# shmurthy08/MoE-GAN_CPSC541

Measured on AMD Instinct MI355X. Metric: images/sec (G+D step, 64x64 MS-COCO layout), higher is better.
Workload: dtype bf16; 1 GPU; C2: 64x64, 8 experts top-2, batch 256/GPU, bf16, R1 on; global_batch=256, experts=8, topk=2, parallelism=dp1, world_seen=1, launch=hipGraph replay

## Files before the change

### include/moegan_hip.h

```cpp
#ifndef MOEGAN_HIP_H
#define MOEGAN_HIP_H
#include <stddef.h>
#include <stdint.h>

#ifdef __cplusplus
extern "C" {
#endif

#define MG_OK 0
#define MG_ERR_ARG (-1)
#define MG_ERR_LAUNCH (-2)

#define MG_F32 0
#define MG_BF16 1
#define MG_F32X3 2

#define MG_ACT_NONE 0
#define MG_ACT_LRELU 1
#define MG_ACT_GELU 2
#define MG_ACT_MUL_GELU_GRAD 3
#define MG_ACT_MUL_LRELU_GRAD 4
#define MG_ACT_RSQRT_EPS 5
#define MG_ACT_QUICK_GELU 6
#define MG_ACT_MUL_QUICK_GELU_GRAD 7
// ... 3 lines not shown
  const float* bias;
  const float* scale;
  int32_t scale_shift;
  int64_t scale_ld;
  const float* rowscale;
  int32_t act;
  const void* aux;
  int64_t ld_aux;
  const void* resid;
  int64_t ld_res;
  int32_t accumulate;
  int32_t atomic;
  int32_t remap_lgcin;
  int32_t remap_taps;
  const int32_t* a_idx;
  int32_t a_idx_div;
  const float* a_rowscale;
  int32_t a_gelu;
  const float* addvec;
  int32_t add_shift;
  int64_t add_ld;
  void* out_pre;
  int64_t ld_pre;
} mg_epilogue;

const char* mg_last_error(void);
int mg_version(void);
const char* mg_source_hash(void);

int mg_set_workspace(void* ptr, size_t bytes, void* stream);
int mg_workspace_reserve(size_t bytes, void* stream);
int64_t mg_workspace_bytes(void* stream);
int mg_set_tuning(int key, int value);

int mg_timer_event_create(void** event);
int mg_timer_event_record(void* event, void* stream);
int mg_timer_event_elapsed(void* start, void* stop, float* ms);
int mg_timer_event_destroy(void* event);
int mg_mark(int tag, void* stream);

typedef struct mg_gemm_desc {
  int32_t M, N, K;
  const void* A;
  int64_t lda;
  const void* B;
  int64_t ldb;
// ... 91 lines not shown
int mg_disc_head_sum(const float* P, int B, int Hf, float* out, void* stream);

int mg_disc_head_bwd_data(int dtype, const float* g, int64_t g_bstride, const float* W2, const void* a1, int B, int Hf, int Cf, int out_dtype, void* ga1, void* stream);

int mg_disc_head_bwd_w(int dtype, const float* g, int64_t g_bstride, const void* h1, int B, int Hf, int Cf, float* dW2, void* stream);

int mg_d_loss(const float* img_real, const float* img_fake, const float* tb, const int32_t* perm, int B, int No, int Nf, float* out, float* g_img, float* g_fake, float* g_tb, float* real_out, float* mism_out, float* fake_out, void* stream);

int mg_g_loss(const float* fake, int B, float scale, float* out, float* g, void* stream);

int mg_r1(int dtype, const void* g, int64_t per, int B, float gamma, float* r1, int u_dtype, void* u, void* stream);

int mg_lrelu_mask_mul(int a_dtype, const void* a, int m_dtype, const void* m, int64_t n, int out_dtype, void* out, void* stream);

int mg_segsum(int dtype, const void* X, int64_t ld, int B, int HW, int C, float* out, void* stream);

int mg_modconv_bwd_out(int dtype, int gz_dtype, const void* gz, int64_t ld_gz, const void* z, int64_t ld_z, const void* zsub, int64_t ld_zsub, const float* d, int B, int HW, int Cout, int act, void* gyt, int64_t ld_gyt, float* gdd, void* stream);

int mg_gather_rows(int dtype, const void* src, int64_t lds, const int32_t* idx, int idx_div, const float* rowscale, int n, int C, void* out, int64_t ldo, void* stream);

int mg_scale_bc(int dtype, const void* x, int64_t ldx, const float* s, int64_t lds, int B, int HW, int C, void* out, int64_t ldo, void* stream);

int mg_modconv_bwd_in(int gxt_dtype, const void* gxt, int64_t ld_gxt, int dtype, const void* x, int64_t ld_x, const float* s, int64_t ld_s, int B, int HW, int Cin, int gx_dtype, void* gx, int64_t ld_gx, int accumulate, float* gs, void* stream);

int mg_kl_coefs(const float* kl2, int R, float eff_w, float* coef, float* total, void* stream);

int mg_router_reparam(const float* mu, const float* rho, const float* eps, int64_t n, float* W, void* stream);

int mg_router_fwd(int dtype, const void* tok, int64_t ld, int T, int C, const float* Wfc, const float* Lt, int E, int k, int HW, const float* temperature, float anneal, int eval_mode, float* probs, float* zlog, int32_t* topi, float* gate, void* stream);

int mg_moe_dispatch(const int32_t* topi, const float* gate, int T, int k, int E, int bm, int32_t* ws, int32_t* row_off, int32_t* tile_off, int32_t* perm, int32_t* pos_of, float* gate_pos, void* stream);

int mg_moe_combine(int dtype, const void* Y, int64_t ldy, const int32_t* pos_of, const float* gate, int T, int k, int C, const void* resid, int64_t ldr, void* out, int64_t ldo, void* stream);
int mg_moe_combine_scaled(int dtype, const void* Y, int64_t ldy, const int32_t* pos_of, const float* gate, int T, int k, int C, const void* resid, int64_t ldr, void* out, int64_t ldo, const float* s, int64_t lds, int HW, void* xs, int64_t ldxs, void* stream);

int mg_moe_gate_grad(int dtype, int gout_dtype, const void* gout, int64_t ldg, const void* Y, int64_t ldy, const int32_t* pos_of, int T, int k, int C, float* g_gate, void* stream);

int mg_router_bwd(const float* probs, const float* zlog, const int32_t* topi, const float* gate, const float* g_gate, const float* g_probs, const float* g_logits, const float* coef, int T, int E, int k, int HW, const float* temperature, float anneal, float* g_raw, float* gsum, float* g_temp, void* stream);

int mg_moe_token_grad(int dtype, const void* gX, int64_t ldx, const int32_t* pos_of, int T, int k, int C, const float* g_raw, const float* Wfc, int E, int out_dtype, void* out, int64_t ldo, void* stream);

int mg_router_feat_grad(int dtype, const void* tok, int64_t ld, int T, int C, const float* g_raw, int E, float* G1, void* stream);

int mg_grouped_colsum(int dtype, const void* X, int64_t ld, const int32_t* idx, int idx_div, const float* rs, const int32_t* row_off, int G, int N, int max_rows, float* out, void* stream);

int mg_router_kl(const float* mu_f, const float* rho_f, int nf, const float* mu_t, const float* rho_t, int nt, const float* mu_c, const float* rho_c, int nc, float* out, void* stream);
// ... 159 lines not shown
```

### moe-gan_cpsc541_amd/csrc/mg_common.h

```cpp
#pragma once
#include <hip/hip_runtime.h>
#include <stdint.h>

#include <algorithm>
#include <atomic>
#include <string>

#include "../../include/moegan_hip.h"

typedef uint16_t bf16_t;
typedef __bf16 bf16x8_t __attribute__((ext_vector_type(8)));
typedef unsigned short u16x8_t __attribute__((ext_vector_type(8)));
typedef unsigned short u16x4_t __attribute__((ext_vector_type(4)));
typedef float f32x4_t __attribute__((ext_vector_type(4)));

#define MG_DEV __device__ __forceinline__

MG_DEV float bf2f(bf16_t h) { return __uint_as_float(((uint32_t)h) << 16); }
MG_DEV bf16_t f2bf(float f) { return __builtin_bit_cast(bf16_t, (__bf16)f); }

MG_DEV float ldf(const float* p, int64_t i) { return p[i]; }
MG_DEV float ldf(const bf16_t* p, int64_t i) { return bf2f(p[i]); }
MG_DEV void stf(float* p, int64_t i, float v) { p[i] = v; }
MG_DEV void stf(bf16_t* p, int64_t i, float v) { p[i] = f2bf(v); }
// ... 105 lines not shown

void mg_set_error(const std::string& msg);
int mg_check_launch(const char* what);
enum { MG_TUNE_WGRAD_TILE = 0, MG_TUNE_GWGRAD_TILE = 1, MG_TUNE_CONV_TILE = 2, MG_TUNE_GEMM_TILE = 3,
       MG_TUNE_WGRAD_SPLITS = 4, MG_TUNE_NO_SLABS = 5, MG_TUNE_XCD = 6 , MG_TUNE_WGRAD_MODE = 7,
       MG_TUNE_WARP_LDS = 8, MG_TUNE_SHORTK = 9, MG_TUNE_ATOMIC_BLOCKS = 10, MG_TUNE_DETERMINISTIC = 11,
       MG_TUNE_S1_OFF = 12,
       MG_TUNE_D0_STORE = 13,
       MG_TUNE_FFN_BWD_OCC = 14,
       MG_TUNE_WIDE_WGRAD = 15,
       MG_TUNE_NARROW = 16,
       MG_TUNE_NARROW_BLOCKS = 17,
       MG_TUNE_DISPATCH3 = 18,
       MG_TUNE_NARROW_WPX = 19,
       MG_TUNE_GWGRAD_BLOCKS = 20,
       MG_TUNE_BATCH_SPLIT = 21,
       MG_TUNE_GROUPED_SHORTK = 22,
       MG_TUNE_SPLITK_FUSED = 23,
       MG_TUNE_ROUTER_TEAM = 24,
       MG_TUNE_ADAMW_CACHED = 25,
       MG_TUNE_ATOMIC_MINK = 26,
       MG_TUNE_WIDE_BLOCKS = 27,
       MG_TUNE_WGRAD_SLAB_BLOCKS = 28,
       MG_TUNE_COUNT = 29 };
extern std::atomic<int> g_mg_tune[MG_TUNE_COUNT];
inline bool mg_det() { return g_mg_tune[MG_TUNE_DETERMINISTIC].load(std::memory_order_relaxed) != 0; }
void* mg_workspace(size_t bytes, hipStream_t stream);
int* mg_tile_counters(int n, hipStream_t stream);
void* mg_fold_alloc(size_t bytes, hipStream_t stream);
int mg_fold_rows_submit(const mg_fold_rows& r, bool deferred, hipStream_t stream);
int mg_fold_wgrad_submit(const mg_fold_wgrad& r, bool deferred, hipStream_t stream);
inline float* mg_fold_partials(size_t bytes, hipStream_t st, bool* deferred) {
  void* p = mg_fold_alloc(bytes, st);
  *deferred = p != nullptr;
  return reinterpret_cast<float*>(p ? p : mg_workspace(bytes, st));
}

namespace {
__global__ __launch_bounds__(1024) void k_det_fold_rows(const float* __restrict__ part, int nrows, int ncols, int na,
                                                        float* __restrict__ out_a, float* __restrict__ out_b) {
  __shared__ float red[16][64];
  const int cx = threadIdx.x & 63, ry = threadIdx.x >> 6;
  const int i = blockIdx.x * 64 + cx;
  float s = 0.f;
  if (i < ncols)
    for (int r = ry; r < nrows; r += 16) s += part[(int64_t)r * ncols + i];
  red[ry][cx] = s;
// ... 19 lines not shown
}
static inline void mg_det_fold_rows(const float* part, int nrows, int ncols, int na, float* out_a, float* out_b,
                             hipStream_t st) {
  hipLaunchKernelGGL(k_det_fold_rows, dim3((ncols + 63) / 64), dim3(1024), 0, st, part, nrows, ncols, na, out_a, out_b);
}

#define MG_REQUIRE(cond, msg)                       \
  do {                                              \
    if (!(cond)) {                                  \
      mg_set_error(std::string(__func__) + ": " + (msg)); \
      return MG_ERR_ARG;                            \
    }                                               \
  } while (0)

static inline int cdiv(int64_t a, int64_t b) { return (int)((a + b - 1) / b); }

bool mg_conv3_direct_ok(int H, int W, int Cin, int Cout, int KH, int KW, int stride, int pad, bool wgrad);
bool mg_conv3_direct(const void* x, int B, int H, int Cin, const void* wpack, int Cout, const mg_epilogue* e, void* y,
                     int64_t ldy, int y_dtype, hipStream_t st);
bool mg_wgrad3_direct(const void* gy, int64_t ldg, const void* x, int B, int H, int Cin, float** ws_out, int* splits,
                      bool* deferred,
                      hipStream_t st);

bool mg_wgrad_wide(int M, int N, int K, const void* A, int64_t lda, const void* B, int64_t ldb, float* C, int64_t ldc,
                   float alpha, hipStream_t st);
```

### moe-gan_cpsc541_amd/csrc/mg_gemm.h

```cpp
#pragma once
#include <type_traits>

#include "mg_common.h"

namespace mg {


constexpr int NTHREADS = 256;
#ifndef MG_DB_MAX_TILE
#define MG_DB_MAX_TILE 0
#endif
#ifndef MG_NSTAGE
#define MG_NSTAGE 1
#endif
#ifndef MG_EPI_BLOCK_SYNC
#define MG_EPI_BLOCK_SYNC 0
#endif
#ifndef MG_SB2_MAX_TILE
#define MG_SB2_MAX_TILE 0
#endif
#ifndef MG_EPI_PREFETCH
#define MG_EPI_PREFETCH 1
#endif
#ifndef MG_SETPRIO
// ... 570 lines not shown
  }
  MG_DEV int pf_kind() const { return 1; }
  MG_DEV void pf_load(int m, int n, Pf& p) const {
    if (this->rm_mode == 1) m = this->remap_row(m);
    const TO* src = this->aux + (int64_t)m * this->ld_aux + n;
#pragma unroll
    for (int j = 0; j < Base::OV; ++j)
      p.v[j] = *reinterpret_cast<const typename Base::ovec_t*>(src + j * VecOf<TO>::N);
  }
  __attribute__((always_inline)) MG_DEV void vec8(int m, int n, float* v, const Pf* pf = nullptr) const {
    float t[8];
    if (pf) Base::pf_unpack(*pf, t);
    else ld8(this->aux + (int64_t)(this->rm_mode == 1 ? this->remap_row(m) : m) * this->ld_aux + n, t);
#pragma unroll
    for (int j = 0; j < 8; ++j) v[j] *= quick_gelu_grad(t[j]);
    Base::vec8(m, n, v, nullptr);
  }
  MG_DEV void operator()(int m, int n, float v) const {
    const int mm = this->rm_mode == 1 ? this->remap_row(m) : m;
    Base::operator()(m, n, v * quick_gelu_grad(ldf(this->aux, (int64_t)mm * this->ld_aux + n)));
  }
};

struct Grouping {
  int mode;
  int ngroups;
  const int* row_off;
  const int* tile_off;
  int rows_per_group;
  int swz;
  int sub_shift;
};

template <typename T> struct Tile;
template <> struct Tile<bf16_t> { static constexpr int BK = 64, PADK = 0, PADM = 32; };
template <> struct Tile<float> { static constexpr int BK = 32, PADK = 4, PADM = 16; };

#ifndef MG_BK_SMALL
#define MG_BK_SMALL 64
#endif
#ifndef MG_X3_BK
#define MG_X3_BK 64
#endif
template <typename T, bool X3, int BM = 128, int BN = 128> constexpr int tile_bk() {
  return X3 ? (BM * BN <= 64 * 64 ? MG_X3_BK : Tile<bf16_t>::BK)
            : (sizeof(T) == 2 && BM * BN <= 64 * 64) ? MG_BK_SMALL : Tile<T>::BK;
// ... 44 lines not shown
MG_DEV void epi_tile(const f32x4_t (&acc)[BM / 32][BN / 32], void* smem, const EP& ep, int m0, int n0, int Mloc,
                     int N, int mrow_base) {
  constexpr int WM = BM / 2, WN = BN / 2, FM = WM / 16, FN = WN / 16;
  const int tid = threadIdx.x, lane = tid & 63, wid = tid >> 6;
  const int wm = wid >> 1, wn = wid & 1;
  const int fr = lane & 15, fq = lane >> 4;
  constexpr int CSP = WN + 4;
  float* cs = reinterpret_cast<float*>(smem) + wid * 16 * CSP;
  constexpr int NE = (2 * WN + 63) / 64;
  constexpr bool kPf = PF && MG_EPI_PREFETCH && EP::OV == 1 && FM * NE * 4 <= 32;
  const bool pfp = kPf && ep.vec_ok && ep.pf_kind() != 0;
  typename EP::Pf pf[kPf ? FM : 1][kPf ? NE : 1];
  if constexpr (kPf) if (pfp) {
#pragma unroll
    for (int i = 0; i < FM; ++i)
#pragma unroll
      for (int t = 0; t < NE; ++t) {
        const int e = lane + 64 * t;
        const int rr = e / (WN / 8), cc = (e - rr * (WN / 8)) * 8;
        const int m = m0 + wm * WM + i * 16 + rr, n = n0 + wn * WN + cc;
        if (e < 2 * WN && m < Mloc && n + 8 <= N) ep.pf_load(mrow_base + m, n, pf[i][t]);
      }
  }
  __syncthreads();
#pragma unroll
  for (int i = 0; i < FM; ++i) {
    if (MG_EPI_BLOCK_SYNC) __syncthreads();
    else { __builtin_amdgcn_fence(__ATOMIC_SEQ_CST, "wavefront"); __builtin_amdgcn_wave_barrier(); }
#pragma unroll
    for (int j = 0; j < FN; ++j)
#pragma unroll
      for (int r = 0; r < 4; ++r) cs[(fq * 4 + r) * CSP + j * 16 + fr] = acc[i][j][r];
    if (MG_EPI_BLOCK_SYNC) __syncthreads();
    else { __builtin_amdgcn_fence(__ATOMIC_SEQ_CST, "wavefront"); __builtin_amdgcn_wave_barrier(); }
    const int mb = m0 + wm * WM + i * 16, nb = n0 + wn * WN;
    if (kPf && pfp) {
#pragma unroll
      for (int t = 0; t < (kPf ? NE : 0); ++t) {
        const int e = lane + 64 * t;
        const int rr = e / (WN / 8), cc = (e - rr * (WN / 8)) * 8;
        const int m = mb + rr, n = nb + cc;
        if (e >= 2 * WN || m >= Mloc) continue;
        const float* src = cs + rr * CSP + cc;
        if (n + 8 <= N) {
          float v[8];
          f32x4_t a = *reinterpret_cast<const f32x4_t*>(src), b = *reinterpret_cast<const f32x4_t*>(src + 4);
#pragma unroll
          for (int j = 0; j < 4; ++j) { v[j] = a[j]; v[j + 4] = b[j]; }
          ep.vec8(mrow_base + m, n, v, &pf[kPf ? i : 0][kPf ? t : 0]);
        } else {
          for (int j = 0; j < 8 && n + j < N; ++j) ep(mrow_base + m, n + j, src[j]);
        }
      }
    } else if (ep.vec_ok) {
#pragma unroll 1
      for (int e = lane; e < 2 * WN; e += 64) {
        int rr = e / (WN / 8), cc = (e - (e / (WN / 8)) * (WN / 8)) * 8;
        int m = mb + rr, n = nb + cc;
        if (m >= Mloc) continue;
        const float* src = cs + rr * CSP + cc;
        if (n + 8 <= N) {
          float v[8];
          f32x4_t a = *reinterpret_cast<const f32x4_t*>(src), b = *reinterpret_cast<const f32x4_t*>(src + 4);
#pragma unroll
          for (int j = 0; j < 4; ++j) { v[j] = a[j]; v[j + 4] = b[j]; }
          ep.vec8(mrow_base + m, n, v);
        } else {
          for (int j = 0; j < 8 && n + j < N; ++j) ep(mrow_base + m, n + j, src[j]);
        }
      }
    } else {
#pragma unroll 1
      for (int e = lane; e < 16 * WN; e += 64) {
        int rr = e / WN, cc = e - (e / WN) * WN;
        int m = mb + rr, n = nb + cc;
        if (m < Mloc && n < N) ep(mrow_base + m, n, cs[rr * CSP + cc]);
      }
    }
  }
}

template <typename T, int BM, int BN, bool A_KC, bool B_KC, class AL, class BL, class EP, bool X3 = false,
          bool PF = false>
MG_DEV void gemm_tile(const AL& A, const BL& B, const EP& ep, int m0, int n0, int Mloc, int N, int kbeg, int kend,
                      int mrow_base) {
  static_assert(!X3 || std::is_same<T, float>::value, "split-bf16 staging takes fp32 operands");
  constexpr int VEC = VecOf<T>::N;
  typedef typename VecOf<T>::type vec_t;
  typedef typename std::conditional<X3, bf16_t, T>::type LT;
  constexpr int TBK = tile_bk<T, X3, BM, BN>();
  constexpr int LDK = TBK + Tile<LT>::PADK;
  constexpr bool GMC = [] {
    if constexpr (!A_KC && !B_KC)
      return MG_GLDS_MC && !X3 && sizeof(T) == 2 && BM == BN && (BM == 64 || BM == 128) && TBK == 64 &&
             has_gldsmc<AL>::value && has_gldsmc<BL>::value;
    else return false;
  }();
  constexpr int PADMC = GMC ? 0 : Tile<LT>::PADM;
  constexpr int LDA = A_KC ? LDK : BM + PADMC;
  constexpr int LDB = B_KC ? LDK : BN + PADMC;
  constexpr int A_ELEMS = A_KC ? BM * LDK : TBK * LDA;
// ... 589 lines not shown
```

### moe-gan_cpsc541_amd/csrc/mg_gemm.hip

```cpp
#include <algorithm>
#include <string>
#include <type_traits>

#include "mg_gemm.h"
#include "mg_host.h"

using namespace mg;

namespace {


constexpr Grouping kNoGroup{0, 1, nullptr, nullptr, 0};
inline Grouping xcd_group() {
  Grouping g = kNoGroup;
  const int x = g_mg_tune[MG_TUNE_XCD];
  g.swz = x == 0 ? 1 : x == 3 ? 0 : x;
  return g;
}

inline bool a_xf(const mg_epilogue* e) { return e && (e->a_idx || e->a_rowscale || e->a_gelu); }

template <typename T, typename TO, int BM, int BN, bool AK, bool BKc, bool XF, bool X3 = false>
void run_plain(int M, int N, int K, const void* A, int64_t lda, const void* B, int64_t ldb, void* C, int64_t ldc,
               const mg_epilogue* e, int splits, hipStream_t st) {
// ... 133 lines not shown

}

extern "C" int mg_gemm(int dtype, int M, int N, int K, const void* A, int64_t lda, int a_kc, const void* B,
                       int64_t ldb, int b_kc, void* C, int64_t ldc, int c_dtype, const mg_epilogue* ep, int splits,
                       void* stream) {
  MG_REQUIRE(dtype == MG_F32 || dtype == MG_BF16 || dtype == MG_F32X3, "bad dtype");
  MG_REQUIRE(M >= 0 && N >= 0 && K >= 0, "negative size");
  if (M == 0 || N == 0) return MG_OK;
  const bool qgg = ep && ep->act == MG_ACT_MUL_QUICK_GELU_GRAD;
  MG_REQUIRE(!qgg || (dtype == MG_BF16 && c_dtype == MG_BF16 && a_kc && !b_kc && splits <= 1 && ep->aux &&
                      !ep->bias && !ep->scale && !ep->out_pre && !ep->atomic && !ep->remap_taps && !a_xf(ep)),
             "MG_ACT_MUL_QUICK_GELU_GRAD: bf16 g [M,K] x W [K,N] -> bf16 with aux, no bias / scale / out_pre / atomic");
  const bool x3 = dtype == MG_F32X3;
  if (x3) dtype = MG_F32;
  const int vec = dtype == MG_F32 ? 4 : 8;
  MG_REQUIRE(aligned16(A) && aligned16(B), "A/B must be 16-byte aligned");
  MG_REQUIRE(lda % vec == 0 && ldb % vec == 0, "lda/ldb must be multiples of the 16-byte vector");
  MG_REQUIRE(a_kc ? (K % vec == 0) : (M % vec == 0), "A vector dim must be a multiple of the 16-byte vector");
  MG_REQUIRE(b_kc ? (K % vec == 0) : (N % vec == 0), "B vector dim must be a multiple of the 16-byte vector");
  MG_REQUIRE(under2g((a_kc ? (int64_t)M : K) * lda, dtype) && under2g((b_kc ? (int64_t)N : K) * ldb, dtype) &&
                 under2g((int64_t)M * ldc, c_dtype),
             "an operand exceeds 2 GiB (32-bit buffer offsets)");
  if (splits < 1 && dtype == MG_BF16 && !x3 && !a_kc && !b_kc && c_dtype == MG_F32 && ep && ep->atomic &&
      !ep->bias && !ep->scale && !ep->rowscale && !ep->act && !ep->aux && !ep->resid && !ep->accumulate &&
      !ep->remap_taps && !ep->a_idx && !ep->a_rowscale && !ep->a_gelu && !ep->addvec && !ep->out_pre &&
      mg_wgrad_wide(M, N, K, A, lda, B, ldb, reinterpret_cast<float*>(C), ldc, ep->alpha,
                    reinterpret_cast<hipStream_t>(stream)))
    return mg_check_launch("mg_gemm (wide weight gradient)");
  if (splits < 1) {
    if (ep && ep->atomic) {
      int64_t tiles = (int64_t)cdiv(M, 64) * cdiv(N, 64);
      const int target = g_mg_tune[MG_TUNE_ATOMIC_BLOCKS] > 0 ? (int)g_mg_tune[MG_TUNE_ATOMIC_BLOCKS] : 512;
      int64_t want = std::max<int64_t>(1, target / std::max<int64_t>(tiles, 1));
      const int mink = g_mg_tune[MG_TUNE_ATOMIC_MINK] > 0 ? (int)g_mg_tune[MG_TUNE_ATOMIC_MINK] : 256;
      splits = (int)std::max<int64_t>(1, std::min<int64_t>(want, K / mink));
    } else {
      splits = 1;
    }
  }
  MG_REQUIRE(splits == 1 || (ep && ep->atomic && c_dtype == MG_F32), "split-K requires an atomic fp32 epilogue");
  MG_REQUIRE(!(ep && ep->atomic) || c_dtype == MG_F32, "atomic epilogue requires fp32 C");
  if (K == 0) splits = 1;
  hipStream_t st = reinterpret_cast<hipStream_t>(stream);
  if (splits > 1 && mg_det()) {
    bool done;
// ... 259 lines not shown
  }
  const bool short_k = KH * KW * Cin <= 256 && M >= 16384;
  if (tile == 128 || (tile == 0 && !short_k && cdiv(M, 128) * (int64_t)cdiv(Cout, 128) >= 480 && Cout > 64))
    run_conv<T, TO, 128, 128>(x, B, H, W, Cin, wpack, Cout, KH, KW, stride, pad, sc, y, ldy, e, st);
  else
    run_conv<T, TO, 64, 64>(x, B, H, W, Cin, wpack, Cout, KH, KW, stride, pad, sc, y, ldy, e, st);
}
}

extern "C" int mg_conv2d_fwd(int dtype, const void* x, int B, int H, int W, int Cin, const void* wpack, int Cout,
                             int KH, int KW, int stride, int pad, const float* in_scale, void* y, int64_t ldy,
                             int y_dtype, const mg_epilogue* ep, void* stream) {
  MG_REQUIRE(dtype == MG_F32 || dtype == MG_BF16, "bad dtype");
  MG_REQUIRE(Cin >= 8 && pow2(Cin), "Cin must be a power of two >= 8");
  int OH = (H + 2 * pad - KH) / stride + 1, OW = (W + 2 * pad - KW) / stride + 1;
  MG_REQUIRE(pow2(H) && pow2(W) && pow2(OH) && pow2(OW), "spatial sizes must be powers of two");
  MG_REQUIRE(aligned16(x) && aligned16(wpack), "x/wpack must be 16-byte aligned");
  MG_REQUIRE(!(ep && ep->atomic) || y_dtype == MG_F32, "atomic epilogue requires fp32 output");
  MG_REQUIRE(under2g((int64_t)B * H * W * Cin, dtype) && under2g((int64_t)Cout * KH * KW * Cin, dtype) &&
                 under2g((int64_t)B * OH * OW * ldy, y_dtype),
             "an operand exceeds 2 GiB (32-bit buffer offsets)");
  if (B == 0) return MG_OK;
  hipStream_t st = reinterpret_cast<hipStream_t>(stream);
  if (dtype == MG_F32) {
    if (y_dtype == MG_F32) run_conv_tiles<float, float>(x, B, H, W, Cin, wpack, Cout, KH, KW, stride, pad, in_scale, y, ldy, ep, st);
    else run_conv_tiles<float, bf16_t>(x, B, H, W, Cin, wpack, Cout, KH, KW, stride, pad, in_scale, y, ldy, ep, st);
  } else {
    if (y_dtype == MG_F32) run_conv_tiles<bf16_t, float>(x, B, H, W, Cin, wpack, Cout, KH, KW, stride, pad, in_scale, y, ldy, ep, st);
    else run_conv_tiles<bf16_t, bf16_t>(x, B, H, W, Cin, wpack, Cout, KH, KW, stride, pad, in_scale, y, ldy, ep, st);
  }
  return mg_check_launch("mg_conv2d_fwd");
}

namespace {
template <typename T, int BM, int BN, bool XF = false>
void run_wgrad(const void* gy, int64_t ldg, const void* x, int B, int H, int W, int Cin, const float* sc, int Cout,
               int KH, int KW, int stride, int pad, float* gw, int splits, hipStream_t st) {
  int OH = (H + 2 * pad - KH) / stride + 1, OW = (W + 2 * pad - KW) / stride + 1;
  int P = B * OH * OW, N = KH * KW * Cin;
  LdMC<T> la{reinterpret_cast<const T*>(gy), ldg, Cout, P, nullptr, 1, nullptr, 0};
  LdMCConv<T, XF> lb{reinterpret_cast<const T*>(x), H, W, Cin, ilog2(Cin), ilog2(OW), ilog2(OH * OW), P,
                     KW, stride, pad, N, sc};
  mg_epilogue e{};
  e.alpha = 1.f;
  e.atomic = 1;
  e.remap_lgcin = ilog2(Cin);
// ... 306 lines not shown
```

### moe-gan_cpsc541_amd/moegan_mi/_lib.py

```python
import ctypes
import os

import torch

_HERE = os.path.dirname(os.path.abspath(__file__))
LIB_PATH = os.environ.get("MOEGAN_HIP_LIB") or os.path.join(_HERE, "libmoegan_hip.so")

MG_F32, MG_BF16 = 0, 1
PREP_PACK, PREP_PACK_FLIP, PREP_PACK_DGRAD_S2, PREP_WSQ, PREP_WSQ_BWD, PREP_REPARAM = 1, 2, 3, 4, 5, 6
ACT_NONE, ACT_LRELU, ACT_GELU, ACT_MUL_GELU_GRAD, ACT_MUL_LRELU_GRAD, ACT_RSQRT_EPS, ACT_QUICK_GELU = range(7)
ACT_MUL_QUICK_GELU_GRAD = 7

_c_void_p, _i32, _i64, _f32 = ctypes.c_void_p, ctypes.c_int32, ctypes.c_int64, ctypes.c_float


class Epilogue(ctypes.Structure):
    _fields_ = [("alpha", _f32), ("bias", _c_void_p), ("scale", _c_void_p), ("scale_shift", _i32),
                ("scale_ld", _i64), ("rowscale", _c_void_p), ("act", _i32), ("aux", _c_void_p),
                ("ld_aux", _i64), ("resid", _c_void_p), ("ld_res", _i64), ("accumulate", _i32),
                ("atomic", _i32), ("remap_lgcin", _i32), ("remap_taps", _i32), ("a_idx", _c_void_p),
                ("a_idx_div", _i32), ("a_rowscale", _c_void_p), ("a_gelu", _i32), ("addvec", _c_void_p),
                ("add_shift", _i32), ("add_ld", _i64), ("out_pre", _c_void_p), ("ld_pre", _i64)]


class GemmDesc(ctypes.Structure):
    _fields_ = [("M", _i32), ("N", _i32), ("K", _i32), ("A", _c_void_p), ("lda", _i64), ("B", _c_void_p),
                ("ldb", _i64), ("C", _c_void_p), ("ldc", _i64), ("ep", ctypes.POINTER(Epilogue))]


class PrepDesc(ctypes.Structure):
    _fields_ = [("kind", _i32), ("Cout", _i32), ("Cin", _i32), ("KH", _i32), ("KW", _i32), ("rows", _i32),
                ("n", _i64), ("W", _c_void_p), ("aux", _c_void_p), ("aux2", _c_void_p), ("out", _c_void_p)]


class ColsumDesc(ctypes.Structure):
    _fields_ = [("dtype", _i32), ("R", _i32), ("C", _i32), ("ld", _i64), ("X", _c_void_p), ("out", _c_void_p)]


class WnDesc(ctypes.Structure):
    _fields_ = [("O", _i32), ("K", _i32), ("v", _c_void_p), ("g", _c_void_p), ("norm", _c_void_p), ("W", _c_void_p),
                ("gW", _c_void_p), ("gv", _c_void_p), ("gg", _c_void_p)]


class RouterParamDesc(ctypes.Structure):
    _fields_ = [("mu", _c_void_p), ("rho", _c_void_p), ("eps", _c_void_p), ("gW", _c_void_p), ("kl_coef", _c_void_p),
# ... 168 lines not shown
        raise MGError(f"{name} failed ({rc}): {lib().mg_last_error().decode()}")


def ptr(t):
    if t is None:
        return None
    return ctypes.c_void_p(t.data_ptr())


def stream():
    return ctypes.c_void_p(torch.cuda.current_stream().cuda_stream)


def dt(t):
    if t.dtype == torch.float32:
        return MG_F32
    if t.dtype == torch.bfloat16:
        return MG_BF16
    raise MGError(f"unsupported dtype {t.dtype}")


def epilogue(alpha=1.0, bias=None, scale=None, scale_shift=0, scale_ld=0, rowscale=None, act=0, aux=None,
             ld_aux=0, resid=None, ld_res=0, accumulate=0, atomic=0, remap_lgcin=0, remap_taps=0, a_idx=None,
             a_idx_div=1, a_rowscale=None, a_gelu=0, addvec=None, add_shift=0, add_ld=0, out_pre=None, ld_pre=0):
    e = Epilogue(alpha, ptr(bias), ptr(scale), scale_shift, scale_ld, ptr(rowscale), act, ptr(aux), ld_aux,
                 ptr(resid), ld_res, accumulate, atomic, remap_lgcin, remap_taps, ptr(a_idx), a_idx_div,
                 ptr(a_rowscale), a_gelu, ptr(addvec), add_shift, add_ld, ptr(out_pre), ld_pre)
    e._keep = (bias, scale, rowscale, aux, resid, a_idx, a_rowscale, addvec, out_pre)
    return e
```

### moe-gan_cpsc541_amd/moegan_mi/engine_g.py

```python
import os

import torch

from . import _lib as L
from . import graphs, ops
from .layout import gen_blocks, max_res_of, rgb_layers

E_ = ops.E
LRELU, GELU, RSQRT = L.ACT_LRELU, L.ACT_GELU, L.ACT_RSQRT_EPS
MUL_GELU_GRAD, MUL_LRELU_GRAD = L.ACT_MUL_GELU_GRAD, L.ACT_MUL_LRELU_GRAD


def _modconv_prefixes(max_res=16):
    out = []
    for name, cin, cout, _, _, attn in gen_blocks(max_res):
        cb = name + ".conv_block."
        out += [(cb + "mtm1.modulated_conv.", 3), (cb + "mtm2.modulated_conv.", 3)]
        if cin != cout:
            out.append((cb + "skip_proj.", 1))
        if attn:
            out += [(name + ".attn_block.proj_in.", 1), (name + ".attn_block.proj_out.", 1)]
    out += [(n + ".", 1) for n, _ in rgb_layers(max_res)[-2:]]
    return out

# ... 141 lines not shown
        else:
            y = ops.conv2d(xs, pk["w"], rows, k, k, 1, k // 2, ep=ep, out_dtype=self.cdt)
        if not save:
            sv = None
        elif ypre is not None:
            sv = (x, xs, w, s, s2, d, ypre, None, 2)
        else:
            sv = (x, xs, w, s, s2, d, y, resid, act)
        return y, sv

    def mc_bwd(self, pre, sv, gz, gx, gw, accumulate=0, gx_f32=False):
        x, xs, w, s, s2, d, z, zsub, act = sv
        B, H, W, Cin = x.shape
        HW = H * W
        pk = self.packs[pre]
        rows = pk["rows"]
        Wt = self.P(pre + "weight")
        Cout, k = Wt.shape[0], Wt.shape[-1]
        P = B * HW
        gyt = torch.empty(P, rows, device=self.dev, dtype=self.cdt)
        gdd = torch.empty(B, rows, device=self.dev, dtype=torch.float32)
        ops.modconv_bwd_out(gz.view(P, -1), z.view(P, -1), d, B, HW, rows, act, gyt, gdd,
                            zsub=None if zsub is None else zsub.view(P, -1))
        if k == 3 and "wflipq" in pk:
            gq, gsc = ops.quant_mx8(gyt)
            gxt = ops.conv2d_mx8(gq.view(B, H, W, rows), gsc, *pk["wflipq"], Cin, 3, 3, 1, 1, out_dtype=self.cdt)
        elif k == 3:
            gxt = ops.conv2d(gyt.view(B, H, W, rows), pk["wflip"], Cin, 3, 3, 1, 1,
                             out_dtype=torch.float32 if gx_f32 else None)
        else:
            gxt = ops.gemm(gyt, pk["w"], P, Cin, rows, b_kc=False)
        batched = self._GS is not None and pre in self.style_cols
        if batched:
            c = self.style_cols[pre]
            gs = self._GS[:, c:c + Cin]
        else:
            gs = ops.zeros(B, Cin, device=self.dev)
        ops.modconv_bwd_in(gxt.view(P, Cin), x.view(P, Cin), s, B, HW, Cin,
                           None if gx is None else gx.view(P, -1), gs, accumulate)
        gW = self.G(pre + "weight")
        if rows == Cout:
            self.side.run(lambda: ops.conv2d_wgrad(gyt, xs, Cout, k, k, 1, k // 2, gW), gyt, xs)
        else:
            def wgrad_padded():
                tmp = ops.zeros(rows, Cin, k, k, device=self.dev)
                ops.conv2d_wgrad(gyt, xs, rows, k, k, 1, k // 2, tmp)
                ops.fold_add([(tmp[:Cout], gW)])
            self.side.run(wgrad_padded, gyt, xs)
        if batched:
            self._demod_bwd.append((pre, gdd, s2, s, gs, Cin, rows, Cout))
            return
        gwsq = ops.gemm(gdd, s2, rows, Cin, B, a_kc=False, b_kc=False)
        self.side.join()
        ops.wsq_bwd(Wt, gwsq[:Cout], self.G(pre + "weight"))
        ops.gemm(gdd, pk["wsq"], B, Cin, rows, b_kc=False, out=gs,
                 ep=E_(alpha=2.0, scale=s, scale_ld=s.stride(0), accumulate=1))
        ops.linear_wgrad(gs, w, self.G(pre + "modulation.weight"))
        ops.colsum(gs, self.G(pre + "modulation.bias"), defer=True)
        ops.gemm(gs, self.P(pre + "modulation.weight"), B, w.shape[1], Cin, b_kc=False, out=gw,
                 ep=E_(accumulate=1))

    def mtm_fwd(self, pre, x, w, resid=None, save=True):
# ... 725 lines not shown
```

### moe-gan_cpsc541_amd/moegan_mi/ops.py

```python
import ctypes
import math

import os

import torch

from . import _lib as L

call, ptr, dt, S = L.call, L.ptr, L.dt, L.stream
E = L.epilogue


TUNE_DETERMINISTIC = 11


def set_deterministic(on=True):
    call("mg_set_tuning", TUNE_DETERMINISTIC, 1 if on else 0)


def _ld(t):
    return t.stride(0) if t.dim() > 1 else t.shape[0]


TIMER = None
# ... 571 lines not shown
         ptr(zsub), zsub.shape[-1] if zsub is not None else 0, ptr(d), B, HW, Cout, act, ptr(gyt),
         ld_gyt or gyt.shape[-1], ptr(gdd), S())


def gather_rows(src, idx, idx_div=1, rowscale=None, out=None):
    n, C = idx.shape[0], src.shape[-1]
    if out is None:
        out = torch.empty(n, C, device=src.device, dtype=src.dtype)
    call("mg_gather_rows", dt(src), ptr(src), _ld(src), ptr(idx), idx_div, ptr(rowscale), n, C, ptr(out), _ld(out), S())
    return out


def scale_bc(x, s, out=None):
    B, C = x.shape[0], x.shape[-1]
    HW = x.numel() // (B * C)
    if out is None:
        out = torch.empty_like(x)
    call("mg_scale_bc", dt(x), ptr(x), C, ptr(s), s.stride(0), B, HW, C, ptr(out), C, S())
    return out


def modconv_bwd_in(gxt, x, s, B, HW, Cin, gx, gs, accumulate=0):
    assert s.stride(0) == gs.stride(0) and s.stride(-1) == 1 and gs.stride(-1) == 1
    call("mg_modconv_bwd_in", dt(gxt), ptr(gxt), gxt.shape[-1], dt(x), ptr(x), x.shape[-1], ptr(s), s.stride(0), B, HW,
         Cin, dt(gx) if gx is not None else 0, ptr(gx), gx.shape[-1] if gx is not None else 0, accumulate, ptr(gs),
         S())


def layernorm_fwd(x, gamma, beta, eps=1e-5, act=0, out=None):
    R, C = x.shape[0], x.shape[-1]
    out = torch.empty_like(x) if out is None else out
    mean = torch.empty(R, device=x.device, dtype=torch.float32)
    rstd = torch.empty(R, device=x.device, dtype=torch.float32)
    call("mg_layernorm_fwd", dt(x), ptr(x), x.shape[-1], R, C, ptr(gamma), ptr(beta), eps, ptr(out), out.shape[-1],
         ptr(mean), ptr(rstd), act, S())
    return out, mean, rstd


def layernorm_bwd(gy, x, mean, rstd, gamma, gx, ggamma, gbeta, accumulate=0):
    R, C = x.shape[0], x.shape[-1]
    call("mg_layernorm_bwd", dt(x), dt(gy), ptr(gy), gy.shape[-1], ptr(x), x.shape[-1], R, C, ptr(mean), ptr(rstd),
         ptr(gamma), ptr(gx), gx.shape[-1] if gx is not None else 0, accumulate, ptr(ggamma), ptr(gbeta), S())


def attn_fwd(qkv, B, L, C, heads=8):
    out = torch.empty(B * L, C, device=qkv.device, dtype=qkv.dtype)
    lse = torch.empty(B, heads, L, device=qkv.device, dtype=torch.float32)
    call("mg_attn_fwd", dt(qkv), ptr(qkv), B, L, C, heads, ptr(out), ptr(lse), S())
    return out, lse
# ... 363 lines not shown
```

Before: 32330 images/sec.

## Fuse modulated-conv input-gradient and style-gradient reduction into data-gradient GEMM epilogue

```diff
diff --git a/include/moegan_hip.h b/include/moegan_hip.h
--- a/include/moegan_hip.h
+++ b/include/moegan_hip.h
@@ -49,6 +49,10 @@
   int64_t add_ld;
   void* out_pre;
   int64_t ld_pre;
+  float* gs;
+  int64_t gs_ld;
+  const void* gs_x;
+  int64_t ld_gs_x;
 } mg_epilogue;
 
 const char* mg_last_error(void);
@@ -186,6 +190,8 @@
 int mg_scale_bc(int dtype, const void* x, int64_t ldx, const float* s, int64_t lds, int B, int HW, int C, void* out, int64_t ldo, void* stream);
 
 int mg_modconv_bwd_in(int gxt_dtype, const void* gxt, int64_t ld_gxt, int dtype, const void* x, int64_t ld_x, const float* s, int64_t ld_s, int B, int HW, int Cin, int gx_dtype, void* gx, int64_t ld_gx, int accumulate, float* gs, void* stream);
+
+int mg_modconv_dgrad_fusable(int dtype, int gx_dtype, int k, int B, int H, int W, int Cout, int Cin, const float* s, int64_t ld_s, const void* x, int64_t ld_x, const void* gx, int64_t ld_gx);
 
 int mg_kl_coefs(const float* kl2, int R, float eff_w, float* coef, float* total, void* stream);
 
diff --git a/moe-gan_cpsc541_amd/csrc/mg_common.h b/moe-gan_cpsc541_amd/csrc/mg_common.h
--- a/moe-gan_cpsc541_amd/csrc/mg_common.h
+++ b/moe-gan_cpsc541_amd/csrc/mg_common.h
@@ -151,7 +151,8 @@
        MG_TUNE_ATOMIC_MINK = 26,
        MG_TUNE_WIDE_BLOCKS = 27,
        MG_TUNE_WGRAD_SLAB_BLOCKS = 28,
-       MG_TUNE_COUNT = 29 };
+       MG_TUNE_MODGRAD_UNFUSED = 29,
+       MG_TUNE_COUNT = 30 };
 extern std::atomic<int> g_mg_tune[MG_TUNE_COUNT];
 inline bool mg_det() { return g_mg_tune[MG_TUNE_DETERMINISTIC].load(std::memory_order_relaxed) != 0; }
 void* mg_workspace(size_t bytes, hipStream_t stream);
@@ -217,5 +218,10 @@
                       bool* deferred,
                       hipStream_t st);
 
+int mg_modgrad_gemm(int dtype, int M, int N, int K, const void* A, int64_t lda, const void* B, int64_t ldb, void* C,
+                    int64_t ldc, int c_dtype, const mg_epilogue* e, hipStream_t st);
+int mg_modgrad_conv(int dtype, const void* x, int B, int H, int W, int Cin, const void* wpack, int Cout, void* y,
+                    int64_t ldy, int y_dtype, const mg_epilogue* e, hipStream_t st);
+
 bool mg_wgrad_wide(int M, int N, int K, const void* A, int64_t lda, const void* B, int64_t ldb, float* C, int64_t ldc,
                    float alpha, hipStream_t st);
diff --git a/moe-gan_cpsc541_amd/csrc/mg_gemm.h b/moe-gan_cpsc541_amd/csrc/mg_gemm.h
--- a/moe-gan_cpsc541_amd/csrc/mg_gemm.h
+++ b/moe-gan_cpsc541_amd/csrc/mg_gemm.h
@@ -616,6 +616,32 @@
   }
 };
 
+template <typename TO, typename TX>
+struct EpiModGrad : Epi<TO> {
+  typedef Epi<TO> Base;
+  static constexpr bool kColSum = true;
+  float* gs; int64_t gs_ld;
+  const TX* gs_x; int64_t ld_gs_x;
+  bool host_vec_ok() const {
+    return Base::host_vec_ok() && this->scale && (reinterpret_cast<uintptr_t>(gs_x) & 15) == 0 && ld_gs_x % 8 == 0;
+  }
+  int round_gxt;
+  MG_DEV void xprod8(int m, int n, float* v, float* p) const {
+    if (round_gxt) {
+#pragma unroll
+      for (int j = 0; j < 8; ++j) v[j] = bf2f(f2bf(v[j]));
+    }
+    float t[8];
+    ld8(gs_x + (int64_t)m * ld_gs_x + n, t);
+#pragma unroll
+    for (int j = 0; j < 8; ++j) p[j] = v[j] * t[j];
+  }
+  MG_DEV int image(int m) const { return m >> this->scale_shift; }
+  MG_DEV void gs_add(int b, int n, float v) const { atomicAdd(gs + (int64_t)b * gs_ld + n, v); }
+};
+template <class EP, class = void> struct has_colsum : std::false_type {};
+template <class EP> struct has_colsum<EP, std::void_t<decltype(EP::kColSum)>> : std::integral_constant<bool, EP::kColSum> {};
+
 struct Grouping {
   int mode;
   int ngroups;
@@ -706,6 +732,22 @@
         if (e < 2 * WN && m < Mloc && n + 8 <= N) ep.pf_load(mrow_base + m, n, pf[i][t]);
       }
   }
+  constexpr bool CSUM = has_colsum<EP>::value;
+  constexpr int NCS = CSUM ? (WN + 63) / 64 : 1;
+  float csum[NCS];
+  int cs_img = -1;
+  auto cs_flush = [&]() {
+    if constexpr (CSUM) {
+#pragma unroll
+      for (int t = 0; t < NCS; ++t) {
+        const int c = lane + 64 * t, n = n0 + wn * WN + c;
+        if (c < WN && n < N) ep.gs_add(cs_img, n, csum[t]);
+      }
+    }
+  };
+  (void)csum;
+  (void)cs_img;
+  (void)cs_flush;
   __syncthreads();
 #pragma unroll
   for (int i = 0; i < FM; ++i) {
@@ -748,9 +790,39 @@
           f32x4_t a = *reinterpret_cast<const f32x4_t*>(src), b = *reinterpret_cast<const f32x4_t*>(src + 4);
 #pragma unroll
           for (int j = 0; j < 4; ++j) { v[j] = a[j]; v[j + 4] = b[j]; }
+          if constexpr (CSUM) {
+            float p[8];
+            ep.xprod8(mrow_base + m, n, v, p);
+            float* dst = cs + rr * CSP + cc;
+            *reinterpret_cast<f32x4_t*>(dst) = f32x4_t{p[0], p[1], p[2], p[3]};
+            *reinterpret_cast<f32x4_t*>(dst + 4) = f32x4_t{p[4], p[5], p[6], p[7]};
+          }
           ep.vec8(mrow_base + m, n, v);
         } else {
           for (int j = 0; j < 8 && n + j < N; ++j) ep(mrow_base + m, n + j, src[j]);
+        }
+      }
+      if constexpr (CSUM) {
+        __builtin_amdgcn_fence(__ATOMIC_SEQ_CST, "wavefront");
+        __builtin_amdgcn_wave_barrier();
+        if (mb < Mloc) {
+          const int img = ep.image(mrow_base + mb), nr = min(16, Mloc - mb);
+          if (img != cs_img) {
+            if (cs_img >= 0) cs_flush();
+            cs_img = img;
+#pragma unroll
+            for (int t = 0; t < NCS; ++t) csum[t] = 0.f;
+          }
+#pragma unroll
+          for (int t = 0; t < NCS; ++t) {
+            const int c = lane + 64 * t;
+            if (c < WN && nb + c < N) {
+              float s = 0.f;
+#pragma unroll
+              for (int rr = 0; rr < 16; ++rr) s += rr < nr ? cs[rr * CSP + c] : 0.f;
+              csum[t] += s;
+            }
+          }
         }
       }
     } else {
@@ -761,6 +833,9 @@
         if (m < Mloc && n < N) ep(mrow_base + m, n, cs[rr * CSP + cc]);
       }
     }
+  }
+  if constexpr (CSUM) {
+    if (cs_img >= 0) cs_flush();
   }
 }
 
diff --git a/moe-gan_cpsc541_amd/csrc/mg_gemm.hip b/moe-gan_cpsc541_amd/csrc/mg_gemm.hip
--- a/moe-gan_cpsc541_amd/csrc/mg_gemm.hip
+++ b/moe-gan_cpsc541_amd/csrc/mg_gemm.hip
@@ -179,6 +179,10 @@
   MG_REQUIRE(under2g((a_kc ? (int64_t)M : K) * lda, dtype) && under2g((b_kc ? (int64_t)N : K) * ldb, dtype) &&
                  under2g((int64_t)M * ldc, c_dtype),
              "an operand exceeds 2 GiB (32-bit buffer offsets)");
+  if (ep && ep->gs) {
+    MG_REQUIRE(a_kc && !b_kc && !x3 && splits <= 1, "mg_epilogue.gs: gyt [M, K] x W [K, N], bf16 or fp32, no split-K");
+    return mg_modgrad_gemm(dtype, M, N, K, A, lda, B, ldb, C, ldc, c_dtype, ep, reinterpret_cast<hipStream_t>(stream));
+  }
   if (splits < 1 && dtype == MG_BF16 && !x3 && !a_kc && !b_kc && c_dtype == MG_F32 && ep && ep->atomic &&
       !ep->bias && !ep->scale && !ep->rowscale && !ep->act && !ep->aux && !ep->resid && !ep->accumulate &&
       !ep->remap_taps && !ep->a_idx && !ep->a_rowscale && !ep->a_gelu && !ep->addvec && !ep->out_pre &&
@@ -484,6 +488,10 @@
              "an operand exceeds 2 GiB (32-bit buffer offsets)");
   if (B == 0) return MG_OK;
   hipStream_t st = reinterpret_cast<hipStream_t>(stream);
+  if (ep && ep->gs) {
+    MG_REQUIRE(KH == 3 && KW == 3 && stride == 1 && pad == 1 && !in_scale, "mg_epilogue.gs: 3x3 / stride 1 / pad 1, no in_scale");
+    return mg_modgrad_conv(dtype, x, B, H, W, Cin, wpack, Cout, y, ldy, y_dtype, ep, st);
+  }
   if (dtype == MG_F32) {
     if (y_dtype == MG_F32) run_conv_tiles<float, float>(x, B, H, W, Cin, wpack, Cout, KH, KW, stride, pad, in_scale, y, ldy, ep, st);
     else run_conv_tiles<float, bf16_t>(x, B, H, W, Cin, wpack, Cout, KH, KW, stride, pad, in_scale, y, ldy, ep, st);
diff --git a/moe-gan_cpsc541_amd/csrc/mg_modgrad.hip b/moe-gan_cpsc541_amd/csrc/mg_modgrad.hip
--- /dev/null
+++ b/moe-gan_cpsc541_amd/csrc/mg_modgrad.hip
@@ -0,0 +1,163 @@
+#include "mg_gemm.h"
+#include "mg_host.h"
+
+using namespace mg;
+
+namespace {
+
+constexpr Grouping kNoGroup{0, 1, nullptr, nullptr, 0};
+
+inline bool unfused_mode() { return mg_det() || g_mg_tune[MG_TUNE_MODGRAD_UNFUSED] != 0; }
+
+inline int gemm_tile_pick(bool bf16, int M, int N, int K) {
+  const int tile = g_mg_tune[MG_TUNE_GEMM_TILE];
+  if (tile == 0 && (K <= (bf16 ? Tile<bf16_t>::BK : Tile<float>::BK) || (K <= 256 && M >= 16384))) return 64;
+  if (bf16 && (tile == 257 || (tile == 0 && N % 256 == 0 && (int64_t)cdiv(M, 128) * (N / 256) >= 480))) return 257;
+  return (tile == 128 || (tile == 0 && (int64_t)cdiv(M, 128) * cdiv(N, 128) >= 480)) ? 128 : 64;
+}
+inline bool gemm_slabs(bool bf16, int M, int N, int K) {
+  if (g_mg_tune[MG_TUNE_NO_SLABS]) return false;
+  const int tbk = bf16 ? tile_bk<bf16_t, false, 64, 64>() : tile_bk<float, false, 64, 64>();
+  const int64_t tiles = (int64_t)cdiv(M, 64) * cdiv(N, 64);
+  if (tiles >= 96 || K < 4 * tbk) return false;
+  return std::min<int64_t>(256 / tiles, K / (2 * tbk)) >= 2;
+}
+inline int conv_tile_pick(bool bf16, int M, int Cout) {
+  const int tile = g_mg_tune[MG_TUNE_CONV_TILE];
+  if (bf16 && (tile == 257 || (tile == 0 && Cout % 256 == 0 && cdiv(M, 128) * (int64_t)(Cout / 256) >= 480))) return 257;
+  return (tile == 128 || (tile == 0 && cdiv(M, 128) * (int64_t)cdiv(Cout, 128) >= 480 && Cout > 64)) ? 128 : 64;
+}
+inline bool conv_slabs(bool bf16, int M, int Cout, int K) {
+  if (g_mg_tune[MG_TUNE_NO_SLABS]) return false;
+  const bool narrow = bf16 && Cout <= 32;
+  const int tbk = bf16 ? tile_bk<bf16_t, false, 64, 64>() : tile_bk<float, false, 64, 64>();
+  const int64_t tiles = (int64_t)cdiv(M, narrow ? 128 : 64) * cdiv(Cout, narrow ? 32 : 64);
+  const int ksteps = K / tbk;
+  if (tiles >= 1024 || ksteps < 16) return false;
+  return std::min<int64_t>(cdiv(1024, tiles), ksteps / 8) >= 2;
+}
+
+const char* refuse(int dtype, int gx_dtype, int k, int B, int H, int W, int Cg, int Cin, const float* s, int64_t ld_s,
+                   const void* x, int64_t ld_x, const void* gx, int64_t ld_gx) {
+  const bool bf16 = dtype == MG_BF16;
+  if (unfused_mode()) return "deterministic mode / MG_TUNE_MODGRAD_UNFUSED";
+  if (dtype != MG_BF16 && dtype != MG_F32) return "operands must be bf16 or fp32";
+  if (gx_dtype != MG_F32 && !(bf16 && gx_dtype == MG_BF16)) return "gx must be fp32, or bf16 with bf16 operands";
+  if (k != 1 && k != 3) return "1x1 or 3x3 only";
+  const int64_t HW = (int64_t)H * W, M = (int64_t)B * HW;
+  if (B < 1 || HW < 16 || !pow2((int)HW) || M >= (1ll << 31)) return "HW must be a power of two >= 16";
+  if (Cin % 8 || Cg % 8) return "channels must be multiples of 8";
+  if (!s || !x || !gx || !aligned16(s) || !aligned16(x) || !aligned16(gx) || ld_s % 4 || ld_x % 8 || ld_gx % 8)
+    return "s / x / gx must be 16-byte aligned with pitches that keep rows so";
+  if (k == 1) {
+    if (gemm_slabs(bf16, (int)M, Cin, Cg)) return "the unfused GEMM runs as split-K slabs";
+  } else {
+    if (!pow2(H) || !pow2(W) || !pow2(Cg)) return "3x3: H, W and the gradient's channels must be powers of two";
+    if (Cg < (bf16 ? max_tile_bk<bf16_t>() : max_tile_bk<float>())) return "3x3: gradient channels below one K step";
+    if (bf16 && mg_conv3_direct_ok(H, W, Cg, Cin, 3, 3, 1, 1, false)) return "the unfused conv runs direct";
+    if (conv_slabs(bf16, (int)M, Cin, 9 * Cg)) return "the unfused conv runs as split-K slabs";
+    if (bf16 && Cin <= 32 && M >= 32768 && g_mg_tune[MG_TUNE_CONV_TILE] == 0) return "the unfused conv runs on 128 x 32 tiles";
+    if (g_mg_tune[MG_TUNE_CONV_TILE] == 256) return "256 x 128 tiles are not built fused";
+  }
+  return nullptr;
+}
+
+const char* refuse_epi(const mg_epilogue* e) {
+  if (!e || !e->gs || !e->gs_x || !e->scale) return "gs, gs_x and scale must be set";
+  if (e->alpha != 1.f || e->bias || e->rowscale || e->act || e->aux || e->resid || e->atomic || e->remap_taps ||
+      e->a_idx || e->a_rowscale || e->a_gelu || e->addvec || e->out_pre)
+    return "no other epilogue step goes with gs";
+  return nullptr;
+}
+
+template <typename TO, typename TX>
+EpiModGrad<TO, TX> make_modgrad(void* C, int64_t ldc, const mg_epilogue* e, bool gemm) {
+  EpiModGrad<TO, TX> ep{make_epi<TO>(C, ldc, e)};
+  ep.round_gxt = sizeof(TX) == 2 && (gemm || sizeof(TO) == 2);
+  ep.gs = e->gs;
+  ep.gs_ld = e->gs_ld;
+  ep.gs_x = reinterpret_cast<const TX*>(e->gs_x);
+  ep.ld_gs_x = e->ld_gs_x;
+  return ep;
+}
+
+template <typename T, typename TO, int BM, int BN>
+bool run_gemm(int M, int N, int K, const void* A, int64_t lda, const void* B, int64_t ldb, void* C, int64_t ldc,
+              const mg_epilogue* e, hipStream_t st) {
+  auto ep = make_modgrad<TO, T>(C, ldc, e, true);
+  if (!ep.host_vec_ok()) return false;
+  LdKC<T> la{reinterpret_cast<const T*>(A), lda, M, K, nullptr, 1, nullptr, 0};
+  LdMC<T> lb{reinterpret_cast<const T*>(B), ldb, N, K, nullptr, 1, nullptr, 0};
+  launch_gemm<T, BM, BN, true, false>(la, lb, ep, M, N, K, 1, kNoGroup, 0, st);
+  return true;
+}
+
+template <typename T, typename TO, int BM, int BN>
+bool run_conv(const void* x, int B, int H, int W, int Cin, const void* wpack, int Cout, void* y, int64_t ldy,
+              const mg_epilogue* e, hipStream_t st) {
+  const int M = B * H * W, K = 9 * Cin;
+  auto ep = make_modgrad<TO, T>(y, ldy, e, false);
+  if (!ep.host_vec_ok()) return false;
+  LdKCConv<T> la{reinterpret_cast<const T*>(x), H, W, Cin, ilog2(Cin), ilog2(W), ilog2(H * W), M, 3, 1, 1, K,
+                 nullptr, kwinv(3)};
+  LdKC<T> lb{reinterpret_cast<const T*>(wpack), K, Cout, K, nullptr, 1, nullptr, 0};
+  launch_gemm<T, BM, BN, true, true>(la, lb, ep, M, Cout, K, 1, kNoGroup, 0, st);
+  return true;
+}
+
+}
+
+extern "C" int mg_modconv_dgrad_fusable(int dtype, int gx_dtype, int k, int B, int H, int W, int Cout, int Cin,
+                                        const float* s, int64_t ld_s, const void* x, int64_t ld_x, const void* gx,
+                                        int64_t ld_gx) {
+  return refuse(dtype, gx_dtype, k, B, H, W, Cout, Cin, s, ld_s, x, ld_x, gx, ld_gx) ? 0 : 1;
+}
+
+#define MG_MODGRAD_REQUIRE(why)                                                     \
+  do {                                                                              \
+    if (const char* w_ = (why)) {                                                   \
+      mg_set_error(std::string(__func__) + ": not covered (" + w_ + "): run the data gradient and mg_modconv_bwd_in"); \
+      return MG_ERR_ARG;                                                            \
+    }                                                                               \
+  } while (0)
+
+int mg_modgrad_gemm(int dtype, int M, int N, int K, const void* A, int64_t lda, const void* B, int64_t ldb, void* C,
+                    int64_t ldc, int c_dtype, const mg_epilogue* e, hipStream_t st) {
+  MG_MODGRAD_REQUIRE(refuse_epi(e));
+  const int HW = 1 << e->scale_shift;
+  MG_REQUIRE(e->scale_shift >= 0 && e->scale_shift < 31 && M % HW == 0, "M must be whole images of 1 << scale_shift pixels");
+  MG_MODGRAD_REQUIRE(refuse(dtype, c_dtype, 1, M / HW, HW, 1, K, N, e->scale, e->scale_ld, e->gs_x, e->ld_gs_x, C, ldc));
+  const bool bf16 = dtype == MG_BF16;
+  const int tile = gemm_tile_pick(bf16, M, N, K);
+  bool ok;
+#define RUN_(T, TO)                                                                                   \
+  (tile == 257 ? run_gemm<T, TO, 128, (sizeof(T) == 2 ? 256 : 128)>(M, N, K, A, lda, B, ldb, C, ldc, e, st) \
+   : tile == 128 ? run_gemm<T, TO, 128, 128>(M, N, K, A, lda, B, ldb, C, ldc, e, st)                  \
+                 : run_gemm<T, TO, 64, 64>(M, N, K, A, lda, B, ldb, C, ldc, e, st))
+  if (!bf16) ok = RUN_(float, float);
+  else if (c_dtype == MG_F32) ok = RUN_(bf16_t, float);
+  else ok = RUN_(bf16_t, bf16_t);
+#undef RUN_
+  MG_REQUIRE(ok, "operands not aligned for the vector epilogue");
+  return mg_check_launch("mg_gemm (modulated-conv data gradient, gx / gs in the epilogue)");
+}
+
+int mg_modgrad_conv(int dtype, const void* x, int B, int H, int W, int Cin, const void* wpack, int Cout, void* y,
+                    int64_t ldy, int y_dtype, const mg_epilogue* e, hipStream_t st) {
+  MG_MODGRAD_REQUIRE(refuse_epi(e));
+  MG_REQUIRE(e->scale_shift == ilog2(H * W) && pow2(H * W), "scale_shift must be log2(H * W)");
+  MG_MODGRAD_REQUIRE(refuse(dtype, y_dtype, 3, B, H, W, Cin, Cout, e->scale, e->scale_ld, e->gs_x, e->ld_gs_x, y, ldy));
+  const bool bf16 = dtype == MG_BF16;
+  const int tile = conv_tile_pick(bf16, B * H * W, Cout);
+  bool ok;
+#define RUN_(T, TO)                                                                                      \
+  (tile == 257 ? run_conv<T, TO, 128, (sizeof(T) == 2 ? 256 : 128)>(x, B, H, W, Cin, wpack, Cout, y, ldy, e, st) \
+   : tile == 128 ? run_conv<T, TO, 128, 128>(x, B, H, W, Cin, wpack, Cout, y, ldy, e, st)                 \
+                 : run_conv<T, TO, 64, 64>(x, B, H, W, Cin, wpack, Cout, y, ldy, e, st))
+  if (!bf16) ok = RUN_(float, float);
+  else if (y_dtype == MG_F32) ok = RUN_(bf16_t, float);
+  else ok = RUN_(bf16_t, bf16_t);
+#undef RUN_
+  MG_REQUIRE(ok, "operands not aligned for the vector epilogue");
+  return mg_check_launch("mg_conv2d_fwd (modulated-conv data gradient, gx / gs in the epilogue)");
+}
diff --git a/moe-gan_cpsc541_amd/moegan_mi/_lib.py b/moe-gan_cpsc541_amd/moegan_mi/_lib.py
--- a/moe-gan_cpsc541_amd/moegan_mi/_lib.py
+++ b/moe-gan_cpsc541_amd/moegan_mi/_lib.py
@@ -20,7 +20,8 @@
                 ("ld_aux", _i64), ("resid", _c_void_p), ("ld_res", _i64), ("accumulate", _i32),
                 ("atomic", _i32), ("remap_lgcin", _i32), ("remap_taps", _i32), ("a_idx", _c_void_p),
                 ("a_idx_div", _i32), ("a_rowscale", _c_void_p), ("a_gelu", _i32), ("addvec", _c_void_p),
-                ("add_shift", _i32), ("add_ld", _i64), ("out_pre", _c_void_p), ("ld_pre", _i64)]
+                ("add_shift", _i32), ("add_ld", _i64), ("out_pre", _c_void_p), ("ld_pre", _i64),
+                ("gs", _c_void_p), ("gs_ld", _i64), ("gs_x", _c_void_p), ("ld_gs_x", _i64)]
 
 
 class GemmDesc(ctypes.Structure):
@@ -235,9 +236,11 @@
 
 def epilogue(alpha=1.0, bias=None, scale=None, scale_shift=0, scale_ld=0, rowscale=None, act=0, aux=None,
              ld_aux=0, resid=None, ld_res=0, accumulate=0, atomic=0, remap_lgcin=0, remap_taps=0, a_idx=None,
-             a_idx_div=1, a_rowscale=None, a_gelu=0, addvec=None, add_shift=0, add_ld=0, out_pre=None, ld_pre=0):
+             a_idx_div=1, a_rowscale=None, a_gelu=0, addvec=None, add_shift=0, add_ld=0, out_pre=None, ld_pre=0,
+             gs=None, gs_ld=0, gs_x=None, ld_gs_x=0):
     e = Epilogue(alpha, ptr(bias), ptr(scale), scale_shift, scale_ld, ptr(rowscale), act, ptr(aux), ld_aux,
                  ptr(resid), ld_res, accumulate, atomic, remap_lgcin, remap_taps, ptr(a_idx), a_idx_div,
-                 ptr(a_rowscale), a_gelu, ptr(addvec), add_shift, add_ld, ptr(out_pre), ld_pre)
-    e._keep = (bias, scale, rowscale, aux, resid, a_idx, a_rowscale, addvec, out_pre)
+                 ptr(a_rowscale), a_gelu, ptr(addvec), add_shift, add_ld, ptr(out_pre), ld_pre, ptr(gs), gs_ld,
+                 ptr(gs_x), ld_gs_x)
+    e._keep = (bias, scale, rowscale, aux, resid, a_idx, a_rowscale, addvec, out_pre, gs, gs_x)
     return e
diff --git a/moe-gan_cpsc541_amd/moegan_mi/engine_g.py b/moe-gan_cpsc541_amd/moegan_mi/engine_g.py
--- a/moe-gan_cpsc541_amd/moegan_mi/engine_g.py
+++ b/moe-gan_cpsc541_amd/moegan_mi/engine_g.py
@@ -187,22 +187,20 @@
         gdd = torch.empty(B, rows, device=self.dev, dtype=torch.float32)
         ops.modconv_bwd_out(gz.view(P, -1), z.view(P, -1), d, B, HW, rows, act, gyt, gdd,
                             zsub=None if zsub is None else zsub.view(P, -1))
-        if k == 3 and "wflipq" in pk:
-            gq, gsc = ops.quant_mx8(gyt)
-            gxt = ops.conv2d_mx8(gq.view(B, H, W, rows), gsc, *pk["wflipq"], Cin, 3, 3, 1, 1, out_dtype=self.cdt)
-        elif k == 3:
-            gxt = ops.conv2d(gyt.view(B, H, W, rows), pk["wflip"], Cin, 3, 3, 1, 1,
-                             out_dtype=torch.float32 if gx_f32 else None)
-        else:
-            gxt = ops.gemm(gyt, pk["w"], P, Cin, rows, b_kc=False)
         batched = self._GS is not None and pre in self.style_cols
         if batched:
             c = self.style_cols[pre]
             gs = self._GS[:, c:c + Cin]
         else:
             gs = ops.zeros(B, Cin, device=self.dev)
-        ops.modconv_bwd_in(gxt.view(P, Cin), x.view(P, Cin), s, B, HW, Cin,
-                           None if gx is None else gx.view(P, -1), gs, accumulate)
+        gx2 = None if gx is None else gx.view(P, -1)
+        if k == 3 and "wflipq" in pk:
+            gq, gsc = ops.quant_mx8(gyt)
+            gxt = ops.conv2d_mx8(gq.view(B, H, W, rows), gsc, *pk["wflipq"], Cin, 3, 3, 1, 1, out_dtype=self.cdt)
+            ops.modconv_bwd_in(gxt.view(P, Cin), x.view(P, Cin), s, B, HW, Cin, gx2, gs, accumulate)
+        else:
+            ops.modconv_bwd_data(gyt, pk["wflip"] if k == 3 else pk["w"], k, B, H, W, Cin, x.view(P, Cin), s, gx2, gs,
+                                 accumulate, gxt_f32=gx_f32)
         gW = self.G(pre + "weight")
         if rows == Cout:
             self.side.run(lambda: ops.conv2d_wgrad(gyt, xs, Cout, k, k, 1, k // 2, gW), gyt, xs)
diff --git a/moe-gan_cpsc541_amd/moegan_mi/ops.py b/moe-gan_cpsc541_amd/moegan_mi/ops.py
--- a/moe-gan_cpsc541_amd/moegan_mi/ops.py
+++ b/moe-gan_cpsc541_amd/moegan_mi/ops.py
@@ -617,9 +617,44 @@
 
 def modconv_bwd_in(gxt, x, s, B, HW, Cin, gx, gs, accumulate=0):
     assert s.stride(0) == gs.stride(0) and s.stride(-1) == 1 and gs.stride(-1) == 1
-    call("mg_modconv_bwd_in", dt(gxt), ptr(gxt), gxt.shape[-1], dt(x), ptr(x), x.shape[-1], ptr(s), s.stride(0), B, HW,
-         Cin, dt(gx) if gx is not None else 0, ptr(gx), gx.shape[-1] if gx is not None else 0, accumulate, ptr(gs),
+    call("mg_modconv_bwd_in", dt(gxt), ptr(gxt), gxt.stride(0), dt(x), ptr(x), x.stride(0), ptr(s), s.stride(0), B, HW,
+         Cin, dt(gx) if gx is not None else 0, ptr(gx), gx.stride(0) if gx is not None else 0, accumulate, ptr(gs),
          S())
+
+
+TUNE_MODGRAD_UNFUSED = 29
+
+
+def modconv_dgrad_fusable(gyt, k, B, H, W, Cin, x, s, gx):
+    if gx is None:
+        return False
+    return bool(L.lib().mg_modconv_dgrad_fusable(_gdt(gyt), dt(gx), k, B, H, W, gyt.shape[-1], Cin, ptr(s),
+                                                 s.stride(0), ptr(x), x.stride(0), ptr(gx), gx.stride(0)))
+
+
+def modconv_dgrad(gyt, w, k, B, H, W, Cin, x, s, gx, gs, accumulate=0):
+    rows = gyt.shape[-1]
+    ep = E(scale=s, scale_shift=ilog2(H * W), scale_ld=s.stride(0), accumulate=accumulate, gs=gs,
+           gs_ld=gs.stride(0), gs_x=x, ld_gs_x=x.stride(0))
+    if k == 3:
+        call("mg_conv2d_fwd", dt(gyt), ptr(gyt), B, H, W, rows, ptr(w), Cin, 3, 3, 1, 1, None, ptr(gx),
+             gx.stride(0), dt(gx), ep, S())
+    else:
+        call("mg_gemm", _gdt(gyt), B * H * W, Cin, rows, ptr(gyt), rows, 1, ptr(w), _ld(w), 0, ptr(gx),
+             gx.stride(0), dt(gx), ep, 1, S())
+
+
+def modconv_bwd_data(gyt, w, k, B, H, W, Cin, x, s, gx, gs, accumulate=0, gxt_f32=False):
+    if modconv_dgrad_fusable(gyt, k, B, H, W, Cin, x, s, gx):
+        modconv_dgrad(gyt, w, k, B, H, W, Cin, x, s, gx, gs, accumulate)
+        return True
+    P, rows = B * H * W, gyt.shape[-1]
+    if k == 3:
+        gxt = conv2d(gyt.view(B, H, W, rows), w, Cin, 3, 3, 1, 1, out_dtype=torch.float32 if gxt_f32 else None)
+    else:
+        gxt = gemm(gyt, w, P, Cin, rows, b_kc=False)
+    modconv_bwd_in(gxt.view(P, Cin), x, s, B, H * W, Cin, gx, gs, accumulate)
+    return False
 
 
 def layernorm_fwd(x, gamma, beta, eps=1e-5, act=0, out=None):
```

Result: faster. 32880 images/sec, median of 6 (+1.7%).
